# myfavouritekk/vdetlib

Measured on AMD Instinct MI355X. Metric: boxes/sec whole-node (NMS+temporal-conv+link), 300f×10k-box synth; mAP parity, higher is better.
Workload: dtype f32; 1 GPU; configs[1]+[2]: 1 video/GPU, 300 frames x 10000 boxes x 200 classes; per-(frame,class) NMS thresh 0.30 + temporal max-pool w=3 + 3-tap temporal convolution; greedy tubelets: 10 tracks/class (stop < 0.90), IoU-link >= 0.50, spatial max-pool IoU > 0.70 + completion + temporal max-pool; frames=300, boxes=10000, classes=200, scores=rand, parallelism=video-per-gpu x1, 4 distinct videos in flight per GPU

## Files before the change

vdetlib_amd/csrc/graphlists_kernels.hpp:

```cpp
#pragma once
#include <hip/hip_runtime.h>
#include <stdint.h>

#include "nms_kernels.hpp"

namespace vdet {

__device__ __forceinline__ int qreach_slot(const GroupDesc &gd, int g) { return ((gd.box_off >> 8) + g) * 4; }

__global__ __launch_bounds__(256) void row_classes_kernel(const float4 *__restrict__ xbox, const GroupDesc *__restrict__ groups,
                                                          const uint32_t *__restrict__ group_flags, float one_minus_t,
                                                          uint16_t *__restrict__ rowperm, float *__restrict__ qreach)
{
    __shared__ float sw[256];
    __shared__ float sreach[256];
    const int g = blockIdx.x, t = blockIdx.y, tid = threadIdx.x;
    if (!(group_flags[g] & kFlagRegular)) return;
    const GroupDesc gd = groups[g];
    if (t * 256 >= gd.nbox) return;
    const int s = t * 256 + tid;
    const bool valid = s < gd.nbox;
    float wd = 3.0e38f, reach = -3.0e38f;
    if (valid) { const float4 b = xbox[gd.box_off + s]; wd = b.z - b.x; reach = b.x + one_minus_t * ((b.z - b.x) + 1.0f) * 1.001f + 1.0f; }
    sw[tid] = wd;
    __syncthreads();
    int rank = 0;
    for (int j = 0; j < 256; ++j) { const float o = sw[j]; rank += (o < wd || (o == wd && j < tid)) ? 1 : 0; }
    if (valid) rowperm[gd.box_off + t * 256 + rank] = (uint16_t)s;
    sreach[rank] = reach;
    __syncthreads();
    float rc = sreach[tid];
#pragma unroll
    for (int d = 32; d > 0; d >>= 1) rc = fmaxf(rc, __shfl_xor(rc, d, 64));
    if ((tid & 63) == 0) qreach[qreach_slot(gd, g) + 4 * t + (tid >> 6)] = rc;
}

struct ListItem { int32_t group; int32_t tq; };

struct GraphListsParams {
    const float4 *xbox;
    const uint16_t *xord;
    const GroupDesc *groups;
    const uint32_t *group_flags;
    const ListItem *items;
    int nitems;
    float t32, one_minus_t;
    uint32_t *row_deg;
    const float2 *reach_table;
    const uint16_t *rowperm;
    const float *qreach;
    uint16_t *adj;
    uint32_t slot_cap;
    int *status;
    int over_bits;
    uint32_t trash_off;
};

__device__ __forceinline__ void emit_half(uint16_t *__restrict__ adj, uint32_t h, uint32_t boff, const uint16_t *ids, uint32_t *lpos,
                                          const uint16_t myid)
{
    constexpr int kSlots = 4;
// ... 187 lines not shown
```

vdetlib_amd/csrc/nms_kernels.hpp:

```cpp
#pragma once
#include <hip/hip_runtime.h>
#include <stdint.h>

namespace vdet {

struct GroupDesc {
    int32_t box_off;
    int32_t nbox;
    int64_t bits_off;
};

__device__ __host__ __forceinline__ int64_t bit_word(int nbox, int v, int c)
{
    const int W = (nbox + 63) >> 6;
    return ((int64_t)(v >> 6) * W + c) * 64 + (v & 63);
}
__host__ __device__ __forceinline__ int64_t bit_words_of_group(int nbox)
{
    const int64_t W = (nbox + 63) >> 6;
    return W * W * 64;
}

struct TileDesc {
    int32_t group;
// ... 760 lines not shown

struct ProblemRef { int g, N, rb; int64_t sbase, sstride, obase; };

__device__ __forceinline__ ProblemRef decode_problem(int mode, int p, int B, int C, const GroupDesc *groups)
{
    ProblemRef r;
    if (mode == 0) { r.g = p / C; const int c = p - r.g * C; r.sbase = (int64_t)r.g * B * C + c; r.sstride = C; r.obase = (int64_t)p * B; }
    else if (mode == 1 || mode == 3) { r.g = p / C; r.sbase = (int64_t)p * B; r.sstride = 1; r.obase = (int64_t)p * B; }
    else { r.g = p; r.sbase = groups[p].box_off; r.sstride = 1; r.obase = groups[p].box_off; }
    r.N = groups[r.g].nbox;
    r.rb = groups[r.g].box_off;
    return r;
}

__device__ __forceinline__ int xcd_problem(int bid, int nblocks)
{
    const int per = nblocks >> 3;
    return (bid & 7) * per + (bid >> 3);
}

__device__ __forceinline__ unsigned long long match8(uint32_t d, bool valid)
{
    unsigned long long peers = __ballot(valid);
#pragma unroll
    for (int b = 0; b < 8; ++b) {
        const bool bit = (d >> b) & 1u;
        const unsigned long long m = __ballot(valid && bit);
        peers &= bit ? m : ~m;
    }
    return peers;
}

template <int BLOCK, int CPW, bool ARANK>
__device__ __forceinline__ void lsd_sort_problem(const SortParams &prm, const int p, unsigned char *smem)
{
    constexpr int NW = BLOCK / 64;
    uint16_t *keys0 = reinterpret_cast<uint16_t *>(smem);
    uint16_t *src = reinterpret_cast<uint16_t *>(smem + prm.lds_idxa_off);
    uint16_t *dst = reinterpret_cast<uint16_t *>(smem + prm.lds_idxb_off);
    uint32_t *bases = reinterpret_cast<uint32_t *>(smem + prm.lds_base_off);
    uint32_t *tot = bases + NW * 256;
    __shared__ uint32_t swt[4];

    const int tid = threadIdx.x, lane = tid & 63, w = tid >> 6;
    const ProblemRef pr = decode_problem(prm.mode, p, prm.B, prm.C, prm.groups);
    const int N = pr.N;

    if (tid == 0) tot[256] = 0;
    __syncthreads();
    uint32_t nx = 0;
    uint32_t khi[(CPW + 1) / 2];
#pragma unroll
    for (int k = 0; k < (CPW + 1) / 2; ++k) khi[k] = 0xFFFFFFFFu;
    uint32_t raw[CPW];
    uint32_t exb[CPW];
    {
        const int lastv = max(N - 1, 0);
        if (prm.keys) {
#pragma unroll
            for (int k = 0; k < CPW; ++k) raw[k] = prm.keys[pr.sbase + min(tid + k * BLOCK, lastv)];
        } else {
#pragma unroll
            for (int k = 0; k < CPW; ++k) raw[k] = __float_as_uint(prm.scores[pr.sbase + (int64_t)min(tid + k * BLOCK, lastv) * pr.sstride]);
        }
#pragma unroll
        for (int k = 0; k < CPW; ++k) exb[k] = 0u;
        if (prm.excl) {
#pragma unroll
            for (int k = 0; k < CPW; ++k) exb[k] = prm.excl[pr.rb + min(tid + k * BLOCK, lastv)];
        }
    }
#pragma unroll
    for (int k = 0; k < CPW; ++k) {
        const int v = tid + k * BLOCK;
        if (v < N) {
            uint32_t ik;
            bool x = false;
            if (prm.keys) {
                const uint32_t kk = raw[k];
                ik = ~kk;
                x = (kk == 0u);
            } else {
                const float sc = __uint_as_float(raw[k]);
                ik = ~score_key(sc);
                if (prm.use_thr && !(sc > prm.thr)) x = true;
            }
            if (exb[k]) x = true;
            if (x) { ik = 0xFFFFFFFFu; ++nx; }
            keys0[v] = (uint16_t)(ik & 0xFFFFu);
            khi[k >> 1] = (k & 1) ? ((khi[k >> 1] & 0x0000FFFFu) | (ik & 0xFFFF0000u))
                                  : ((khi[k >> 1] & 0xFFFF0000u) | (ik >> 16));
            src[v] = (uint16_t)(N - 1 - v);
        }
    }
    if (nx) atomicAdd(&tot[256], nx);
    __syncthreads();
    const int ncand = N - (int)tot[256];

    const int nchunks = (N + 63) >> 6;
    const int c0 = w * CPW;

    for (int pass = 0; pass < 4; ++pass) {
        const int shift = (pass & 1) * 8;
        if (pass == 2) {
#pragma unroll
            for (int k = 0; k < CPW; ++k) {
                const int v = tid + k * BLOCK;
                if (v < N) keys0[v] = (uint16_t)((k & 1) ? (khi[k >> 1] >> 16) : (khi[k >> 1] & 0xFFFFu));
            }
        }
        for (int i = tid; i < NW * 256; i += BLOCK) bases[i] = 0;
        __syncthreads();
        uint32_t ra[CPW];
        uint32_t rl[CPW];
        bool peel_on = false;
#pragma unroll
        for (int ch = 0; ch < CPW; ++ch) {
            const int q = (c0 + ch) * 64 + lane;
            const bool valid = (c0 + ch) < nchunks && q < N;
            const uint32_t i = valid ? src[q] : 0u;
            const uint32_t d = valid ? (((uint32_t)keys0[i] >> shift) & 255u) : 0u;
            ra[ch] = i | (d << 16);
            if (ARANK) {
                uint32_t r = 0u;
                bool pending = valid;
#pragma unroll
                for (int peel = 0; peel < 2; ++peel) {
                    if (ch > 0 && !peel_on) break;
                    const unsigned long long rem = __ballot(pending);
                    if (rem) {
                        const int l0 = __ffsll((unsigned long long)rem) - 1;
// ... 30 lines not shown
#pragma unroll
            for (int ww = 0; ww < NW; ++ww) dsum += bases[ww * 256 + tid];
            dincl = dsum;
#define VDET_SCAN_STEP(CTRL, ROWMASK) dincl += (uint32_t)__builtin_amdgcn_update_dpp(0, (int)dincl, CTRL, ROWMASK, 0xf, false);
            VDET_SCAN_STEP(0x111, 0xf) VDET_SCAN_STEP(0x112, 0xf) VDET_SCAN_STEP(0x114, 0xf) VDET_SCAN_STEP(0x118, 0xf)
            VDET_SCAN_STEP(0x142, 0xa) VDET_SCAN_STEP(0x143, 0xc)
#undef VDET_SCAN_STEP
            if (lane == 63) swt[w] = dincl;
        }
        __syncthreads();
        if (tid < 256) {
            uint32_t run = dincl - dsum;
            for (int k = 0; k < w; ++k) run += swt[k];
#pragma unroll
            for (int ww = 0; ww < NW; ++ww) {
                const uint32_t c = bases[ww * 256 + tid];
                bases[ww * 256 + tid] = run;
                run += c;
            }
        }
        __syncthreads();
#pragma unroll
        for (int ch = 0; ch < CPW; ++ch) {
            const int q = (c0 + ch) * 64 + lane;
            const bool valid = (c0 + ch) < nchunks && q < N;
            if (valid) {
                const uint32_t d = ra[ch] >> 16;
                dst[bases[w * 256 + d] + rl[ch]] = (uint16_t)(ra[ch] & 0xFFFFu);
            }
        }
        __syncthreads();
        uint16_t *t = src; src = dst; dst = t;
    }
    int ncand_out = ncand;
    if (prm.topk > 0 && ncand > prm.topk) {
        const int k = prm.topk;
        if (w == 0) {
            auto key_at = [&](int q) -> uint32_t {
                const int i = src[q];
                if (prm.keys) return prm.keys[pr.sbase + i];
                return score_key(prm.scores[pr.sbase + (int64_t)i * pr.sstride]);
            };
            const uint32_t kk = key_at(k - 1);
            int a = k - 1, b = k;
            for (;;) {
                const int q = a - 1 - lane;
                const bool eq = q >= 0 && key_at(q) == kk;
                const unsigned long long m = __ballot(eq);
                const int n = m == ~0ull ? 64 : (__ffsll((unsigned long long)~m) - 1);
                a -= n;
                if (n < 64) break;
            }
            for (;;) {
                const int q = b + lane;
                const bool eq = q < ncand && key_at(q) == kk;
                const unsigned long long m = __ballot(eq);
                const int n = m == ~0ull ? 64 : (__ffsll((unsigned long long)~m) - 1);
                b += n;
                if (n < 64) break;
            }
            const int nsel = k - a, s0 = b - nsel;
            if (s0 > a)
                for (int t = 0; t < nsel; t += 64) {
                    const bool v = t + lane < nsel;
                    const uint16_t e = v ? src[s0 + t + lane] : (uint16_t)0;
                    __builtin_amdgcn_fence(__ATOMIC_ACQ_REL, "wavefront");
// ... 574 lines not shown
```

vdetlib_amd/csrc/vdet_capi.hip:

```cpp
#include <hip/hip_runtime.h>
#include <atomic>
#include <chrono>

#include <algorithm>
#include <cmath>
#include <cstdarg>
#include <cstdio>
#include <cstdlib>
#include <cstring>
#include <string>
#include <vector>

#include "../../include/vdet_hip.h"
#include "nms_kernels.hpp"
#include "binsort_kernels.hpp"
#include "small_kernels.hpp"
#include "detnms_kernels.hpp"
#include "fused_kernels.hpp"
#include "adjrows_kernels.hpp"
#include "graphlists_kernels.hpp"
#include "temporal_kernels.hpp"
#include "tubelet_kernels.hpp"
#include "track_kernels.hpp"
#include "batch_kernels.hpp"
#include "gemm_kernels.hpp"
#include "eval_kernels.hpp"
#include "tcn_kernels.hpp"
#include "interp_kernels.hpp"
#include "anchor_kernels.hpp"

using namespace vdet;

namespace {

struct DevBuf {
    void *p = nullptr;
    size_t cap = 0;
    hipError_t reserve(size_t bytes)
    {
        if (bytes <= cap) return hipSuccess;
        if (p) (void)hipFree(p);
        p = nullptr;
        cap = 0;
        size_t want = bytes + bytes / 4 + 256;
        hipError_t e = hipMalloc(&p, want);
        if (e != hipSuccess) {
            want = bytes;
            e = hipMalloc(&p, want);
// ... 70 lines not shown
    size_t bits_budget = (size_t)1 << 30;
    size_t max_lds = 160 * 1024;
    int n_cu = 256;
    DevBuf boxes, scores, keys, excl, frames, groups, tiles, bits, rowz, rowmeta, groupz, adj, comp, origidx,
        out64, trk_frames, trk_boxes, b1, b2, iou_out, order, ncand, keepidx, keepcnt, gflags, pairs, tkeys, tstate, visited, heads, xkeys, xord, wmeta, wmeta16, reachtab, rowperm, qreach, ditems, striptot, stripoff, xncand, xbox, xbox16, xord16, xcum, xinfo, tmp[8];
    bool timing = false;
    bool timing_accumulate = false;
    std::vector<std::pair<hipEvent_t, hipEvent_t>> ev_pool;
    std::vector<int> ev_stage;
    size_t ev_used = 0;
    float last_ms[ST_COUNT] = {0};
    int last_launches[ST_COUNT] = {0};
    bool sort_attr_set = false;
    bool cache_enabled = false;
    struct PrepKey { const void *boxes = nullptr; int64_t F = 0, B = 0; float t32 = 0; ListsKey lists; } prep;
    bool graph_valid = false, lists_valid = false;
    struct KeySrc { const void *scores = nullptr; int64_t F = 0, B = 0, C = 0; int use_thr = 0; float thr = 0; } keysrc;
    bool keys_valid = false;
    bool vpass_attr_set = false;
    bool index_valid = false; const void *index_boxes = nullptr; int64_t index_F = 0, index_B = 0;
    bool all_regular = false;
    bool wave_transpose = false;
    bool no_lazy = false;
    bool no_index = false;
    bool force_general = false;
    bool atomic_rank = false;
    bool small_lists = true;
    bool adj_rows = true;
    bool direct_lists = true;
    uint32_t direct_cap = 384;
    int64_t direct_ntot = 0;
    unsigned long long direct_fixed = 0;
    bool no_fused = false;
    bool binsort = true;
    const std::vector<GroupDesc> *host_groups = nullptr;
    bool sym_built = false;
    NmsPlan vplan;
    bool vplan_valid = false;
    int64_t vplan_F = 0, vplan_B = 0;
    size_t vplan_budget = 0;
    long long n_host_syncs = 0;
    bool async_enabled = false;
    unsigned long long pool_hint = 0;
    bool topk_attr_set = false;
    float gt32 = 0.f;
    bool wmeta16_built = false;
    bool wmeta_built = false;
    bool last_sort_binned = false;
    StagedTab vidtab, segtab;
    DevBuf sortctl;
    DevBuf nover;
    DevBuf ordncand;
    DevBuf linkmemo, linkstats, linkwarm, linkorder, linkchains, linknodes, tracknode, rtodo;
    struct NodeKey { const void *tracks = nullptr, *boxes = nullptr; int64_t F = 0, B = 0, C = 0; int T = 0; double nms_thres = 0; } nodekey;
    bool nodes_valid = false;
    void *fused_in = nullptr, *fused_out = nullptr;
    void *fused_in_dev = nullptr, *fused_out_dev = nullptr;
    void *fbatch_in = nullptr, *fbatch_out = nullptr, *fbatch_in_dev = nullptr, *fbatch_out_dev = nullptr;
    size_t fbatch_in_cap = 0, fbatch_out_cap = 0;
    bool fbatch_attr = false;
    size_t dyn_lds_max = 0;
    DevBuf ev_tab, ev_dtp, ev_dsc, ev_dslot, ev_bcnt, ev_boff, ev_key[2], ev_val[2], ev_hist;
    DevBuf tcn_x, tcn_frames, tcn_base, tcn_len, tcn_scratch;
    StagedTab tcn_params, tcn_foff, tcn_ovtab;
    bool tcn_tiled = false;
    bool tcn_global = false;
// ... 133 lines not shown
        if (gd.nbox < 2) { gd.bits_off = 0; continue; }
        const size_t words = (size_t)bit_words_of_group(gd.nbox);
        if (cur && cur + words > budget_words) {
            pl.batch_tiles.push_back({t0, (int)pl.tiles.size()});
            pl.batch_pairs.push_back({p0, (int)pl.pairs.size()});
            pl.batch_ditems.push_back({d0, (int)pl.ditems.size()});
            t0 = (int)pl.tiles.size();
            p0 = (int)pl.pairs.size();
            d0 = (int)pl.ditems.size();
            pl.bits_words_max = std::max(pl.bits_words_max, cur);
            cur = 0;
        }
        gd.bits_off = (int64_t)cur;
        cur += words;
        const int nrt = (gd.nbox + kRowsPerTile - 1) / kRowsPerTile;
        for (int rt = 0; rt < nrt; ++rt) pl.tiles.push_back({(int32_t)g, rt});
        for (int rt = 0; rt < nrt; ++rt)
            for (int ct = rt; ct < nrt; ++ct) pl.pairs.push_back({(int32_t)g, (int16_t)rt, (int16_t)ct});
        for (int q = 3; q >= 0; --q)
            for (int rt = 0; rt < nrt; ++rt) pl.ditems.push_back({(int32_t)g, (int32_t)(4 * rt + q)});
    }
    if ((int)pl.tiles.size() > t0) {
        pl.batch_tiles.push_back({t0, (int)pl.tiles.size()});
        pl.batch_pairs.push_back({p0, (int)pl.pairs.size()});
        pl.batch_ditems.push_back({d0, (int)pl.ditems.size()});
    }
    pl.bits_words_max = std::max(pl.bits_words_max, cur);
    (void)c;
    return VDET_OK;
}

int sort_groups_by_keys(vdet_ctx *c, int G, int nmax, int64_t ntot);

int build_frame_index(vdet_ctx *c, const float4 *d_boxes, int64_t ntot, int64_t G, int nmax)
{
    if (c->cache_enabled && c->index_valid && c->index_boxes == d_boxes && c->index_F == G && c->index_B == ntot) return VDET_OK;
    c->index_valid = false;
    HIPCHK(c, c->xkeys.reserve((size_t)ntot * 4));
    HIPCHK(c, c->xord.reserve((size_t)ntot * 2));
    HIPCHK(c, c->xncand.reserve((size_t)G * 4));
    HIPCHK(c, c->xbox.reserve((size_t)ntot * 16));
    HIPCHK(c, c->xbox16.reserve((size_t)(ntot + G + 4) * 8));
    HIPCHK(c, c->xord16.reserve((size_t)(ntot + G + 4) * 2));
    HIPCHK(c, c->xcum.reserve((size_t)G * 257 * 4));
    HIPCHK(c, c->xinfo.reserve((size_t)G * 16));
    StageTimer tm(c, ST_OTHER);
    hipLaunchKernelGGL(xkey_kernel, dim3((unsigned)((ntot + 255) / 256)), dim3(256), 0, c->stream, d_boxes,
                       c->xkeys.as<uint32_t>(), ntot);
    int rc = sort_groups_by_keys(c, (int)G, nmax, ntot);
    if (rc) return rc;
    hipLaunchKernelGGL(frame_index_kernel, dim3((unsigned)G), dim3(256), 0, c->stream, d_boxes, c->groups.as<GroupDesc>(),
                       c->xord.as<uint16_t>(), c->xbox.as<float4>(), c->xcum.as<uint32_t>(), c->xinfo.as<float>(),
                       c->gflags.as<uint32_t>(), c->xbox16.as<uint2>(), c->xord16.as<uint16_t>());
    HIPCHK(c, hipGetLastError());
    c->index_valid = true; c->index_boxes = d_boxes; c->index_F = G; c->index_B = ntot;
    return VDET_OK;
}

FrameIndex frame_index_of(vdet_ctx *c)
{
    return FrameIndex{c->xbox.as<float4>(), c->xord.as<uint16_t>(), c->xcum.as<uint32_t>(), c->xinfo.as<float>(),
                      c->xbox16.as<uint2>(), c->xord16.as<uint16_t>(), 0};
}

NmsPlan &volume_plan(vdet_ctx *c, int64_t F, int64_t B)
{
    if (c->vplan_F == F && c->vplan_B == B && c->vplan_budget == c->bits_budget && !c->vplan.groups.empty()) return c->vplan;
    (void)host_sync(c);
    c->graph_valid = c->lists_valid = c->index_valid = c->nodes_valid = false;
    c->vplan = NmsPlan();
    c->vplan.groups.resize((size_t)F);
    for (int64_t f = 0; f < F; ++f) c->vplan.groups[(size_t)f] = {(int32_t)(f * B), (int32_t)B, 0};
    make_plan(c, c->vplan);
    c->vplan_F = F; c->vplan_B = B; c->vplan_budget = c->bits_budget;
    c->vplan_valid = false;
    return c->vplan;
}

int volume_groups(vdet_ctx *c, int64_t F, int64_t B)
{
    NmsPlan &pl = volume_plan(c, F, B);
    c->host_groups = &pl.groups;
    HIPCHK(c, c->groups.reserve((size_t)F * sizeof(GroupDesc)));
    if (!c->vplan_valid)
        HIPCHK(c, hipMemcpyAsync(c->groups.p, pl.groups.data(), (size_t)F * sizeof(GroupDesc), hipMemcpyHostToDevice, c->stream));
    return VDET_OK;
}

// ... 111 lines not shown
        if (!pl.ditems.empty())
            HIPCHK(c, hipMemcpyAsync(c->ditems.p, pl.ditems.data(), pl.ditems.size() * sizeof(ListItem),
                                     hipMemcpyHostToDevice, c->stream));
        HIPCHK(c, hipMemcpyAsync(c->groups.p, pl.groups.data(), G * sizeof(GroupDesc), hipMemcpyHostToDevice, c->stream));
        if (!pl.tiles.empty())
            HIPCHK(c, hipMemcpyAsync(c->tiles.p, pl.tiles.data(), pl.tiles.size() * sizeof(TileDesc),
                                     hipMemcpyHostToDevice, c->stream));
        c->vplan_valid = volume;
    }
    auto direct_now = [&]() {
        return c->direct_lists && c->adj_rows && c->wave_transpose && pl.nmax > 384 && t32 > 1e-30f && t32 < INFINITY && !c->force_general &&
               (size_t)8 * pl.nmax + 24 * 1024 <= c->max_lds && ((unsigned long long)pl.ntot + 1ull) * c->direct_cap * 2ull + 512ull <= 0xFFFFFFFFull;
    };
    auto fixed_pool = [&]() { return direct_now() ? (unsigned long long)pl.ntot * c->direct_cap + std::max<unsigned long long>(c->direct_cap, 128) : 0ull; };
    unsigned long long min_pool = fixed_pool() + (unsigned long long)pl.ntot * (direct_now() ? 1 : 32);
    const bool async = volume && c->async_enabled && c->pool_hint > 0;
    if (async) {
        const unsigned long long dyn_hint = c->pool_hint > fixed_pool() ? c->pool_hint - fixed_pool() : 0ull;
        const unsigned long long want = std::max(min_pool, fixed_pool() + dyn_hint + dyn_hint / 2);
        if (c->adj.cap < want * 2) HIPCHK(c, c->adj.reserve((size_t)want * 2 + 4096));
    } else {
        Counters h0;
        HIPCHK(c, hipMemcpyAsync(&h0, c->d_cnt, sizeof h0, hipMemcpyDeviceToHost, c->stream));
        HIPCHK(c, host_sync(c));
        if (h0.status && !c->latched) c->latched = translate_status(c, h0.status);
        if (h0.eindex && !c->latched) c->latched = fail(c, VDET_EINDEX, "list index out of range");
        if (c->adj.cap < min_pool * 2) HIPCHK(c, c->adj.reserve((size_t)min_pool * 2 + 4096));
    }

    for (int attempt = 0; attempt < 3; ++attempt) {
        const bool direct = direct_now();
        min_pool = fixed_pool() + (unsigned long long)pl.ntot * (direct ? 1 : 32);
        if (!async && c->adj.cap < min_pool * 2) HIPCHK(c, c->adj.reserve((size_t)min_pool * 2 + 4096));
        HIPCHK(c, hipMemsetAsync(c->rowz.p, 0, (size_t)pl.ntot * 4, c->stream));
        HIPCHK(c, hipMemsetAsync(c->rowmeta.p, 0, (size_t)pl.ntot * 8, c->stream));
        HIPCHK(c, hipMemsetAsync(c->groupz.p, 0, G * 4, c->stream));
        if (async) {
            hipLaunchKernelGGL(fold_pool_kernel, dim3(1), dim3(1), 0, c->stream, c->d_cnt);
            HIPCHK(c, hipMemsetAsync((char *)c->d_cnt + kPerBuildOff, 0, sizeof(Counters) - kPerBuildOff, c->stream));
        }
        else HIPCHK(c, hipMemsetAsync(c->d_cnt, 0, sizeof(Counters), c->stream));
        c->direct_ntot = direct ? pl.ntot : 0;
        c->direct_fixed = fixed_pool();
        if (direct) hipLaunchKernelGGL(pool_start_kernel, dim3(1), dim3(1), 0, c->stream, &c->d_cnt->pool_used, fixed_pool());
        const int pool_bits = async ? (kStPool | kStPoolAsync) : kStPool;
        const unsigned long long pool_cap = (c->adj.cap - 2048) / 2;
        const bool use_sym = t32 > 1e-30f && t32 < INFINITY && !c->force_general &&
                             (size_t)8 * pl.nmax + 24 * 1024 <= c->max_lds;
        c->sym_built = use_sym;
        c->wmeta_built = use_sym;
        if (c->wmeta_built) HIPCHK(c, c->wmeta.reserve((size_t)pl.ntot * sizeof(WalkMeta)));
        if (c->wmeta_built && c->adj_rows && pl.nmax > 384) HIPCHK(c, c->wmeta16.reserve((size_t)pl.ntot * sizeof(uint4)));
        if (use_sym) {
            {
                StageTimer tm(c, ST_OTHER);
                hipLaunchKernelGGL(frame_flags_kernel, dim3((unsigned)G), dim3(256), 0, c->stream, d_boxes,
                                   c->groups.as<GroupDesc>(), c->gflags.as<uint32_t>(), &c->d_cnt->irregular);
            }
            if (!volume) c->index_valid = false;
            const int rci = build_frame_index(c, d_boxes, pl.ntot, (int64_t)G, pl.nmax);
            if (rci) return rci;
            HIPCHK(c, c->reachtab.reserve((size_t)(pl.ntot / 64 + (int64_t)G + 2) * sizeof(float2)));
            {
                StageTimer tm(c, ST_OTHER);
                hipLaunchKernelGGL(reach_table_kernel, dim3((unsigned)G), dim3(256), 0, c->stream, c->xbox.as<float4>(),
                                   c->groups.as<GroupDesc>(), c->gflags.as<uint32_t>(), one_minus_t, c->reachtab.as<float2>());
                if (direct) {
                    HIPCHK(c, c->rowperm.reserve((size_t)pl.ntot * 2 + 1024));
                    HIPCHK(c, c->qreach.reserve((size_t)(pl.ntot / 256 + (int64_t)G + 2) * 4 * sizeof(float)));
                    hipLaunchKernelGGL(row_classes_kernel, dim3((unsigned)G, (unsigned)((pl.nmax + 255) / 256)), dim3(256), 0, c->stream,
                                       c->xbox.as<float4>(), c->groups.as<GroupDesc>(), c->gflags.as<uint32_t>(), one_minus_t,
                                       c->rowperm.as<uint16_t>(), c->qreach.as<float>());
                }
            }
        } else {
            c->index_valid = false;
        }
        if (direct && !pl.ditems.empty()) {
            StageTimer tm(c, ST_IOU_BITS);
            GraphListsParams gp;
            gp.xbox = c->xbox.as<float4>(); gp.xord = c->xord.as<uint16_t>(); gp.groups = c->groups.as<GroupDesc>();
            gp.group_flags = c->gflags.as<uint32_t>(); gp.items = c->ditems.as<ListItem>(); gp.nitems = (int)pl.ditems.size();
            gp.t32 = t32; gp.one_minus_t = one_minus_t; gp.row_deg = c->rowz.as<uint32_t>(); gp.reach_table = c->reachtab.as<float2>();
            gp.rowperm = c->rowperm.as<uint16_t>(); gp.qreach = c->qreach.as<float>(); gp.adj = c->adj.as<uint16_t>();
            gp.slot_cap = c->direct_cap; gp.status = &c->d_cnt->status; gp.over_bits = pool_bits | kStDirect;
            gp.trash_off = (uint32_t)((unsigned long long)pl.ntot * c->direct_cap * 2ull);
// ... 608 lines not shown
    if (hipGetDeviceCount(&ndev) != hipSuccess || ndev <= 0) {
        delete c;
        return VDET_EHIP;
    }
    if (device < 0) {
        if (hipGetDevice(&device) != hipSuccess) { delete c; return VDET_EHIP; }
    }
    if (device >= ndev || hipSetDevice(device) != hipSuccess) { delete c; return VDET_EINVAL; }
    c->device = device;
    hipDeviceProp_t prop;
    if (hipGetDeviceProperties(&prop, device) == hipSuccess) {
        c->n_cu = prop.multiProcessorCount > 0 ? prop.multiProcessorCount : 256;
        if (strncmp(prop.gcnArchName, "gfx950", 6) != 0) c->max_lds = 64 * 1024;
    }
    if (const char *e = getenv("VDET_FORCE_GENERAL")) c->force_general = atoi(e) != 0;
    if (const char *e = getenv("VDET_BITS_BUDGET_MB")) {
        const long mb = atol(e);
        if (mb > 0) c->bits_budget = (size_t)mb << 20;
    }
    if (hipStreamCreateWithFlags(&c->own_stream, hipStreamNonBlocking) != hipSuccess ||
        hipMalloc((void **)&c->d_cnt, sizeof(Counters)) != hipSuccess) {
        delete c;
        return VDET_EHIP;
    }
    c->stream = c->own_stream;
    (void)hipMemsetAsync(c->d_cnt, 0, sizeof(Counters), c->stream);
    if (const char *e = getenv("VDET_NO_INDEX")) c->no_index = atoi(e) != 0;
    if (const char *e = getenv("VDET_NO_LAZY")) c->no_lazy = atoi(e) != 0;
    if (const char *e = getenv("VDET_NO_FUSED")) c->no_fused = atoi(e) != 0;
    if (const char *e = getenv("VDET_ADJ_ROWS")) c->adj_rows = atoi(e) != 0;
    if (const char *e = getenv("VDET_DIRECT_LISTS")) c->direct_lists = atoi(e) != 0;
    if (const char *e = getenv("VDET_DIRECT_CAP")) { const int v = atoi(e); if (v >= 8 && v <= 32760) c->direct_cap = (uint32_t)(v & ~7); }
    if (const char *e = getenv("VDET_BINSORT")) c->binsort = atoi(e) != 0;
    if (const char *e = getenv("VDET_SMALL_LISTS")) c->small_lists = atoi(e) != 0;
    if (const char *e = getenv("VDET_TCN_TILED")) c->tcn_tiled = atoi(e) != 0;
    if (const char *e = getenv("VDET_TCN_GLOBAL")) c->tcn_global = atoi(e) != 0;
    {
        const int npat = 4096;
        std::vector<uint8_t> pats((size_t)npat * 64);
        uint32_t rs = 12345u;
        auto rnd = [&]() { rs = rs * 1664525u + 1013904223u; return rs >> 8; };
        for (int t = 0; t < npat; ++t) {
            const int kind = t % 8;
            const int nd = kind == 0 ? 1 : kind == 1 ? 2 : kind == 2 ? 3 : kind == 3 ? 8 : kind == 4 ? 32 : kind == 5 ? 64 : kind == 6 ? 200 : 254;
            for (int l = 0; l < 64; ++l) {
                uint8_t d = (uint8_t)(rnd() % nd);
                if (kind == 7 && (rnd() & 3) == 0) d = 255;
                if (t % 16 == 9) d = (uint8_t)((l * (1 + t % 7)) % nd);
                pats[(size_t)t * 64 + l] = d;
            }
        }
        bool ok = false;
        DevBuf pb;
        if (pb.reserve(pats.size()) == hipSuccess &&
            hipMemcpyAsync(pb.p, pats.data(), pats.size(), hipMemcpyHostToDevice, c->stream) == hipSuccess) {
            hipLaunchKernelGGL(lds_atomic_order_probe, dim3(256), dim3(64), 0, c->stream, pb.as<uint8_t>(), npat,
                               &c->d_cnt->status);
            Counters h;
            if (hipMemcpyAsync(&h, c->d_cnt, sizeof h, hipMemcpyDeviceToHost, c->stream) == hipSuccess &&
                host_sync(c) == hipSuccess)
                ok = (h.status == 0);
        }
        pb.release();
        (void)hipMemsetAsync(c->d_cnt, 0, sizeof(Counters), c->stream);
        c->atomic_rank = ok;
        if (const char *e = getenv("VDET_ATOMIC_RANK")) c->atomic_rank = c->atomic_rank && atoi(e) != 0;
// ... 63 lines not shown
int vdet_reset_stream(vdet_ctx *c)
{
    if (!c) return VDET_EINVAL;
    c->stream = c->own_stream;
    return VDET_OK;
}

const char *vdet_last_error(vdet_ctx *c) { return c ? c->err.c_str() : "null context"; }

int vdet_set_cache(vdet_ctx *c, int enable)
{
    if (!c) return VDET_EINVAL;
    c->cache_enabled = enable != 0;
    c->graph_valid = c->lists_valid = c->index_valid = c->keys_valid = c->nodes_valid = false;
    return VDET_OK;
}

int vdet_invalidate(vdet_ctx *c)
{
    if (!c) return VDET_EINVAL;
    c->graph_valid = c->lists_valid = c->index_valid = c->keys_valid = c->nodes_valid = false;
    return VDET_OK;
}

int vdet_query(vdet_ctx *c, int what)
{
    if (!c) return VDET_EINVAL;
    if (what == 0) return c->atomic_rank ? 1 : 0;
    if (what == 1) return c->n_cu;
    if (what == 2) return c->all_regular ? 1 : 0;
    if (what == 3) return c->wave_transpose ? 1 : 0;
    if (what == 8) return (int)std::min<long long>(c->n_host_syncs, 0x7FFFFFFF);
    if (what == 10) return (int)std::min<long long>(c->tcn_params.uploads, 0x7FFFFFFF);
    if (what == 9) {
        if (!c->last_sort_binned || !c->sortctl.p) return -1;
        BinSortCtl h{};
        if (hipMemcpyAsync(&h, c->sortctl.p, sizeof h, hipMemcpyDeviceToHost, c->stream) != hipSuccess || host_sync(c) != hipSuccess) return VDET_EHIP;
        return h.nfail;
    }
    if (what >= 4 && what <= 7) {
        unsigned int h[4] = {0, 0, 0, 0};
        if (!c->linkstats.p) return 0;
        if (hipMemcpyAsync(h, c->linkstats.p, 16, hipMemcpyDeviceToHost, c->stream) != hipSuccess ||
            host_sync(c) != hipSuccess) return VDET_EHIP;
        return (int)std::min<unsigned int>(h[what - 4], 0x7FFFFFFFu);
    }
    return VDET_EINVAL;
}

int vdet_set_timing(vdet_ctx *c, int enable)
{
    if (!c) return VDET_EINVAL;
    c->timing = enable != 0;
    c->timing_accumulate = enable == 2;
    c->ev_used = 0;
    return VDET_OK;
}

int vdet_last_timing_ms(vdet_ctx *c, float *out16)
{
    float *out8 = out16;
    if (!c || !out8) return VDET_EINVAL;
    HIPCHK(c, host_sync(c));
    for (int i = 0; i < ST_COUNT; ++i) { c->last_ms[i] = 0; c->last_launches[i] = 0; }
    for (size_t i = 0; i < c->ev_used; ++i) {
        float ms = 0;
// ... 1739 lines not shown
```

Baseline: 332.5 million boxes/s.

## Fuse per-frame index build, flags, memsets and row ordering into one prep kernel

Adds a frame_prep_kernel with one 1024-thread block per frame. It computes validity and u16 flags, radix-sorts boxes by x in LDS, writes the sorted xbox/xord/xbox16, the bucket histogram prefix, the reach table, and the rowperm/qreach width ranks. The same kernel zeroes rowz, rowmeta and groupz and does the pool-start/fold bookkeeping, replacing several separate kernels and memsets. The goal is to cut launch count and the repeated global re-reads of boxes, at the cost of large LDS use per block and possibly lower occupancy. The row_classes_kernel rank loop now also runs only over valid entries.

```diff
diff --git a/vdetlib_amd/csrc/frameprep_kernels.hpp b/vdetlib_amd/csrc/frameprep_kernels.hpp
--- /dev/null
+++ b/vdetlib_amd/csrc/frameprep_kernels.hpp
@@ -0,0 +1,212 @@
+#pragma once
+#include <hip/hip_runtime.h>
+#include <stdint.h>
+
+#include "graphlists_kernels.hpp"
+#include "nms_kernels.hpp"
+
+namespace vdet {
+
+constexpr int kPrepBlock = 1024;
+constexpr int kPrepHistWords = 272;
+
+struct FramePrepParams {
+    const float4 *boxes;
+    const GroupDesc *groups;
+    uint32_t *group_flags;
+    int *n_irregular;
+    uint16_t *xord; float4 *xbox; uint32_t *xcum; float *xinfo; uint2 *xbox16; uint16_t *xord16;
+    float2 *reachtab;
+    uint16_t *rowperm; float *qreach;
+    uint32_t *rowz; uint2 *rowmeta; uint32_t *groupz;
+    unsigned long long *pool_used, *pool_max;
+    unsigned long long pool_start;
+    int fold;
+    float one_minus_t;
+    int lds_keys_off, lds_idxb_off, lds_base_off;
+};
+
+__host__ __device__ inline size_t frame_prep_lds(int nmax, int *keys_off, int *idxb_off, int *base_off)
+{
+    const size_t idx = (((size_t)2 * (size_t)(nmax > 1 ? nmax : 1)) + 15) & ~(size_t)15;
+    const size_t widths = (size_t)4 * (((size_t)nmax + 255) & ~(size_t)255);
+    const size_t base = idx + (2 * idx > widths ? 2 * idx : widths);
+    if (keys_off) *keys_off = (int)idx;
+    if (idxb_off) *idxb_off = (int)(2 * idx);
+    if (base_off) *base_off = (int)base;
+    return base + (size_t)4 * ((kPrepBlock / 64) * 256 + 256 + 4);
+}
+
+template <int CPW, bool ARANK>
+__global__ __launch_bounds__(kPrepBlock) void frame_prep_kernel(const FramePrepParams prm)
+{
+    extern __shared__ __attribute__((aligned(16))) unsigned char smem[];
+    constexpr int BLOCK = kPrepBlock;
+    __shared__ float smin[BLOCK / 64], smax[BLOCK / 64], swm[BLOCK / 64];
+    __shared__ uint32_t swsum[4];
+    const int g = blockIdx.x, tid = threadIdx.x, lane = tid & 63, w = tid >> 6;
+    if (g == 0 && tid == 0) {
+        if (prm.fold && *prm.pool_used > *prm.pool_max) *prm.pool_max = *prm.pool_used;
+        *prm.pool_used = prm.pool_start;
+    }
+    const GroupDesc gd = prm.groups[g];
+    const int N = gd.nbox;
+    const int64_t fo = gd.box_off;
+    if (tid == 0) prm.groupz[g] = 0u;
+    if (N <= 0) {
+        if (tid == 0) prm.group_flags[g] = kFlagRegular | kFlagU16;
+        return;
+    }
+    const float4 *fb = prm.boxes + fo;
+    uint16_t *src = reinterpret_cast<uint16_t *>(smem);
+    uint16_t *keys0 = reinterpret_cast<uint16_t *>(smem + prm.lds_keys_off);
+    uint16_t *dst = reinterpret_cast<uint16_t *>(smem + prm.lds_idxb_off);
+    uint32_t *bases = reinterpret_cast<uint32_t *>(smem + prm.lds_base_off);
+
+    constexpr int LD = CPW < 6 ? CPW : 6;
+    uint32_t khi[(CPW + 1) / 2];
+#pragma unroll
+    for (int k = 0; k < (CPW + 1) / 2; ++k) khi[k] = 0xFFFFFFFFu;
+    int bad = 0, wide = 0;
+    float mn = 3.0e38f, mx = -3.0e38f, wm = 0.0f;
+    const float inf = __uint_as_float(0x7F800000u);
+#pragma unroll
+    for (int k0 = 0; k0 < CPW; k0 += LD) {
+        float4 bx[LD];
+#pragma unroll
+        for (int j = 0; j < LD; ++j)
+            if (k0 + j < CPW) bx[j] = fb[min(tid + (k0 + j) * BLOCK, N - 1)];
+#pragma unroll
+        for (int j = 0; j < LD; ++j) {
+            const int k = k0 + j < CPW ? k0 + j : CPW - 1;
+            const int v = tid + k * BLOCK;
+            if (k0 + j < CPW && v < N) {
+                const float4 b = bx[j];
+                const float bw = (b.z - b.x) + 1.0f, bh = (b.w - b.y) + 1.0f;
+                const float a = bw * bh;
+                const bool ok = fabsf(b.x) < inf && fabsf(b.y) < inf && fabsf(b.z) < inf && fabsf(b.w) < inf && bw > 0.0f && bh > 0.0f && a < inf;
+                bad |= ok ? 0 : 1;
+                const bool small = b.x == truncf(b.x) && b.y == truncf(b.y) && b.z == truncf(b.z) && b.w == truncf(b.w) &&
+                                   fmaxf(fmaxf(b.x, b.y), fmaxf(b.z, b.w)) <= 65535.0f &&
+                                   ((__float_as_uint(b.x) | __float_as_uint(b.y) | __float_as_uint(b.z) | __float_as_uint(b.w)) >> 31) == 0u;
+                wide |= small ? 0 : 1;
+                mn = fminf(mn, b.x); mx = fmaxf(mx, b.x); wm = fmaxf(wm, bw);
+                const uint32_t ik = score_key(b.x);
+                keys0[v] = (uint16_t)(ik & 0xFFFFu);
+                khi[k >> 1] = (k & 1) ? ((khi[k >> 1] & 0x0000FFFFu) | (ik & 0xFFFF0000u)) : ((khi[k >> 1] & 0xFFFF0000u) | (ik >> 16));
+                src[v] = (uint16_t)(N - 1 - v);
+                prm.rowz[fo + v] = 0u;
+                prm.rowmeta[fo + v] = make_uint2(0u, 0u);
+            }
+        }
+    }
+#pragma unroll
+    for (int d = 32; d > 0; d >>= 1) {
+        mn = fminf(mn, __shfl_xor(mn, d, 64)); mx = fmaxf(mx, __shfl_xor(mx, d, 64)); wm = fmaxf(wm, __shfl_xor(wm, d, 64));
+    }
+    if (lane == 0) { smin[w] = mn; smax[w] = mx; swm[w] = wm; }
+    const int any_bad = __syncthreads_or(bad);
+    const int any_wide = __syncthreads_or(wide);
+    const uint32_t fl = (any_bad ? 0u : kFlagRegular) | (any_wide ? 0u : kFlagU16);
+    if (tid == 0) {
+        prm.group_flags[g] = fl;
+        if (any_bad) atomicAdd(prm.n_irregular, 1);
+    }
+#pragma unroll
+    for (int i = 0; i < BLOCK / 64; ++i) { mn = fminf(mn, smin[i]); mx = fmaxf(mx, smax[i]); wm = fmaxf(wm, swm[i]); }
+    const float xmin = mn, xmax = mx;
+    const float scale = xmax > xmin ? 256.0f / (xmax - xmin) : 0.0f;
+
+    lsd_sort_passes<BLOCK, CPW, ARANK>(keys0, src, dst, bases, khi, N);
+
+    float *swd = reinterpret_cast<float *>(smem + prm.lds_keys_off);
+    uint32_t *hist = bases;
+    float *sreach = reinterpret_cast<float *>(bases + kPrepHistWords);
+    for (int i = tid; i < 257; i += BLOCK) hist[i] = 0u;
+    __syncthreads();
+    const bool regular = (fl & kFlagRegular) != 0u;
+    const bool u16 = prm.xbox16 && (fl & kFlagU16);
+    const int64_t p16 = pair_pos(fo + g);
+#pragma unroll
+    for (int k = 0; k < CPW; ++k) {
+        const int r = tid + k * BLOCK;
+        float4 b = make_float4(0.f, 0.f, 0.f, 0.f);
+        float reach = -3.0e38f;
+        if (r < N) {
+            const uint16_t o = src[r];
+            b = fb[o];
+            prm.xbox[fo + r] = b;
+            prm.xord[fo + r] = o;
+            if (u16) {
+                prm.xbox16[p16 + r] = make_uint2((uint32_t)b.x | ((uint32_t)b.y << 16), (uint32_t)b.z | ((uint32_t)b.w << 16));
+                prm.xord16[p16 + r] = o;
+            }
+            atomicAdd(&hist[xbucket(b.x, xmin, scale) + 1], 1u);
+            swd[r] = b.z - b.x;
+            reach = b.x + prm.one_minus_t * ((b.z - b.x) + 1.0f) * 1.001f + 1.0f;
+        }
+        const int cb = k * (BLOCK / 64) + w;
+        if (regular && cb * 64 < N) {
+#pragma unroll
+            for (int d = 32; d > 0; d >>= 1) reach = fmaxf(reach, __shfl_xor(reach, d, 64));
+            const float first = __shfl(b.x, 0, 64);
+            if (lane == 0) prm.reachtab[reach_slot(gd, g) + cb] = make_float2(reach, first);
+        }
+    }
+    __syncthreads();
+    {
+        uint32_t incl = 0u;
+        if (tid < 256) {
+            incl = hist[tid + 1];
+#pragma unroll
+            for (int d = 1; d < 64; d <<= 1) { const uint32_t o = __shfl_up(incl, d, 64); if (lane >= d) incl += o; }
+            if (lane == 63) swsum[w] = incl;
+        }
+        __syncthreads();
+        if (tid < 256) {
+            for (int i = 0; i < w; ++i) incl += swsum[i];
+            prm.xcum[(int64_t)g * 257 + tid + 1] = incl;
+        }
+        if (tid == 0) {
+            prm.xcum[(int64_t)g * 257] = 0u;
+            prm.xinfo[g * 4 + 0] = xmin; prm.xinfo[g * 4 + 1] = scale; prm.xinfo[g * 4 + 2] = wm; prm.xinfo[g * 4 + 3] = 0.0f;
+        }
+    }
+
+    if (!prm.rowperm || !regular) return;
+    const int grp = tid >> 8, pos = tid & 255;
+#pragma unroll
+    for (int k = 0; k < CPW; ++k) {
+        if (k * BLOCK < N) {
+            const int tile = grp + 4 * k, tb = tile * 256;
+            const int nv = min(256, N - tb);
+            int rank = pos;
+            float reach = -3.0e38f;
+            if (pos < nv) {
+                const float4 b = prm.xbox[fo + tb + pos];
+                reach = b.x + prm.one_minus_t * ((b.z - b.x) + 1.0f) * 1.001f + 1.0f;
+                const float wd = swd[tb + pos];
+                rank = 0;
+                for (int j = 0; j < nv; j += 4) {
+                    const float4 o = *reinterpret_cast<const float4 *>(swd + tb + j);
+                    rank += (o.x < wd || (o.x == wd && j < pos)) ? 1 : 0;
+                    rank += (j + 1 < nv && (o.y < wd || (o.y == wd && j + 1 < pos))) ? 1 : 0;
+                    rank += (j + 2 < nv && (o.z < wd || (o.z == wd && j + 2 < pos))) ? 1 : 0;
+                    rank += (j + 3 < nv && (o.w < wd || (o.w == wd && j + 3 < pos))) ? 1 : 0;
+                }
+                prm.rowperm[fo + tb + rank] = (uint16_t)(tb + pos);
+            }
+            if (nv > 0) sreach[grp * 256 + rank] = reach;
+            __syncthreads();
+            if (nv > 0) {
+                float rc = sreach[tid];
+#pragma unroll
+                for (int d = 32; d > 0; d >>= 1) rc = fmaxf(rc, __shfl_xor(rc, d, 64));
+                if (lane == 0) prm.qreach[qreach_slot(gd, g) + 4 * tile + (w & 3)] = rc;
+            }
+            __syncthreads();
+        }
+    }
+}
+
+}
diff --git a/vdetlib_amd/csrc/graphlists_kernels.hpp b/vdetlib_amd/csrc/graphlists_kernels.hpp
--- a/vdetlib_amd/csrc/graphlists_kernels.hpp
+++ b/vdetlib_amd/csrc/graphlists_kernels.hpp
@@ -20,13 +20,17 @@
     if (t * 256 >= gd.nbox) return;
     const int s = t * 256 + tid;
     const bool valid = s < gd.nbox;
-    float wd = 3.0e38f, reach = -3.0e38f;
+    float wd = 0.0f, reach = -3.0e38f;
     if (valid) { const float4 b = xbox[gd.box_off + s]; wd = b.z - b.x; reach = b.x + one_minus_t * ((b.z - b.x) + 1.0f) * 1.001f + 1.0f; }
     sw[tid] = wd;
     __syncthreads();
-    int rank = 0;
-    for (int j = 0; j < 256; ++j) { const float o = sw[j]; rank += (o < wd || (o == wd && j < tid)) ? 1 : 0; }
-    if (valid) rowperm[gd.box_off + t * 256 + rank] = (uint16_t)s;
+    const int nv = min(256, gd.nbox - t * 256);
+    int rank = tid;
+    if (valid) {
+        rank = 0;
+        for (int j = 0; j < nv; ++j) { const float o = sw[j]; rank += (o < wd || (o == wd && j < tid)) ? 1 : 0; }
+        rowperm[gd.box_off + t * 256 + rank] = (uint16_t)s;
+    }
     sreach[rank] = reach;
     __syncthreads();
     float rc = sreach[tid];
diff --git a/vdetlib_amd/csrc/nms_kernels.hpp b/vdetlib_amd/csrc/nms_kernels.hpp
--- a/vdetlib_amd/csrc/nms_kernels.hpp
+++ b/vdetlib_amd/csrc/nms_kernels.hpp
@@ -816,71 +816,12 @@
 }
 
 template <int BLOCK, int CPW, bool ARANK>
-__device__ __forceinline__ void lsd_sort_problem(const SortParams &prm, const int p, unsigned char *smem)
+__device__ __forceinline__ void lsd_sort_passes(uint16_t *keys0, uint16_t *&src, uint16_t *&dst, uint32_t *bases, const uint32_t (&khi)[(CPW + 1) / 2],
+                                                const int N)
 {
     constexpr int NW = BLOCK / 64;
-    uint16_t *keys0 = reinterpret_cast<uint16_t *>(smem);
-    uint16_t *src = reinterpret_cast<uint16_t *>(smem + prm.lds_idxa_off);
-    uint16_t *dst = reinterpret_cast<uint16_t *>(smem + prm.lds_idxb_off);
-    uint32_t *bases = reinterpret_cast<uint32_t *>(smem + prm.lds_base_off);
-    uint32_t *tot = bases + NW * 256;
     __shared__ uint32_t swt[4];
-
     const int tid = threadIdx.x, lane = tid & 63, w = tid >> 6;
-    const ProblemRef pr = decode_problem(prm.mode, p, prm.B, prm.C, prm.groups);
-    const int N = pr.N;
-
-    if (tid == 0) tot[256] = 0;
-    __syncthreads();
-    uint32_t nx = 0;
-    uint32_t khi[(CPW + 1) / 2];
-#pragma unroll
-    for (int k = 0; k < (CPW + 1) / 2; ++k) khi[k] = 0xFFFFFFFFu;
-    uint32_t raw[CPW];
-    uint32_t exb[CPW];
-    {
-        const int lastv = max(N - 1, 0);
-        if (prm.keys) {
-#pragma unroll
-            for (int k = 0; k < CPW; ++k) raw[k] = prm.keys[pr.sbase + min(tid + k * BLOCK, lastv)];
-        } else {
-#pragma unroll
-            for (int k = 0; k < CPW; ++k) raw[k] = __float_as_uint(prm.scores[pr.sbase + (int64_t)min(tid + k * BLOCK, lastv) * pr.sstride]);
-        }
-#pragma unroll
-        for (int k = 0; k < CPW; ++k) exb[k] = 0u;
-        if (prm.excl) {
-#pragma unroll
-            for (int k = 0; k < CPW; ++k) exb[k] = prm.excl[pr.rb + min(tid + k * BLOCK, lastv)];
-        }
-    }
-#pragma unroll
-    for (int k = 0; k < CPW; ++k) {
-        const int v = tid + k * BLOCK;
-        if (v < N) {
-            uint32_t ik;
-            bool x = false;
-            if (prm.keys) {
-                const uint32_t kk = raw[k];
-                ik = ~kk;
-                x = (kk == 0u);
-            } else {
-                const float sc = __uint_as_float(raw[k]);
-                ik = ~score_key(sc);
-                if (prm.use_thr && !(sc > prm.thr)) x = true;
-            }
-            if (exb[k]) x = true;
-            if (x) { ik = 0xFFFFFFFFu; ++nx; }
-            keys0[v] = (uint16_t)(ik & 0xFFFFu);
-            khi[k >> 1] = (k & 1) ? ((khi[k >> 1] & 0x0000FFFFu) | (ik & 0xFFFF0000u))
-                                  : ((khi[k >> 1] & 0xFFFF0000u) | (ik >> 16));
-            src[v] = (uint16_t)(N - 1 - v);
-        }
-    }
-    if (nx) atomicAdd(&tot[256], nx);
-    __syncthreads();
-    const int ncand = N - (int)tot[256];
-
     const int nchunks = (N + 63) >> 6;
     const int c0 = w * CPW;
 
@@ -977,6 +918,74 @@
         __syncthreads();
         uint16_t *t = src; src = dst; dst = t;
     }
+}
+
+template <int BLOCK, int CPW, bool ARANK>
+__device__ __forceinline__ void lsd_sort_problem(const SortParams &prm, const int p, unsigned char *smem)
+{
+    constexpr int NW = BLOCK / 64;
+    uint16_t *keys0 = reinterpret_cast<uint16_t *>(smem);
+    uint16_t *src = reinterpret_cast<uint16_t *>(smem + prm.lds_idxa_off);
+    uint16_t *dst = reinterpret_cast<uint16_t *>(smem + prm.lds_idxb_off);
+    uint32_t *bases = reinterpret_cast<uint32_t *>(smem + prm.lds_base_off);
+    uint32_t *tot = bases + NW * 256;
+    const int tid = threadIdx.x, lane = tid & 63, w = tid >> 6;
+    const ProblemRef pr = decode_problem(prm.mode, p, prm.B, prm.C, prm.groups);
+    const int N = pr.N;
+
+    if (tid == 0) tot[256] = 0;
+    __syncthreads();
+    uint32_t nx = 0;
+    uint32_t khi[(CPW + 1) / 2];
+#pragma unroll
+    for (int k = 0; k < (CPW + 1) / 2; ++k) khi[k] = 0xFFFFFFFFu;
+    uint32_t raw[CPW];
+    uint32_t exb[CPW];
+    {
+        const int lastv = max(N - 1, 0);
+        if (prm.keys) {
+#pragma unroll
+            for (int k = 0; k < CPW; ++k) raw[k] = prm.keys[pr.sbase + min(tid + k * BLOCK, lastv)];
+        } else {
+#pragma unroll
+            for (int k = 0; k < CPW; ++k) raw[k] = __float_as_uint(prm.scores[pr.sbase + (int64_t)min(tid + k * BLOCK, lastv) * pr.sstride]);
+        }
+#pragma unroll
+        for (int k = 0; k < CPW; ++k) exb[k] = 0u;
+        if (prm.excl) {
+#pragma unroll
+            for (int k = 0; k < CPW; ++k) exb[k] = prm.excl[pr.rb + min(tid + k * BLOCK, lastv)];
+        }
+    }
+#pragma unroll
+    for (int k = 0; k < CPW; ++k) {
+        const int v = tid + k * BLOCK;
+        if (v < N) {
+            uint32_t ik;
+            bool x = false;
+            if (prm.keys) {
+                const uint32_t kk = raw[k];
+                ik = ~kk;
+                x = (kk == 0u);
+            } else {
+                const float sc = __uint_as_float(raw[k]);
+                ik = ~score_key(sc);
+                if (prm.use_thr && !(sc > prm.thr)) x = true;
+            }
+            if (exb[k]) x = true;
+            if (x) { ik = 0xFFFFFFFFu; ++nx; }
+            keys0[v] = (uint16_t)(ik & 0xFFFFu);
+            khi[k >> 1] = (k & 1) ? ((khi[k >> 1] & 0x0000FFFFu) | (ik & 0xFFFF0000u))
+                                  : ((khi[k >> 1] & 0xFFFF0000u) | (ik >> 16));
+            src[v] = (uint16_t)(N - 1 - v);
+        }
+    }
+    if (nx) atomicAdd(&tot[256], nx);
+    __syncthreads();
+    const int ncand = N - (int)tot[256];
+
+    lsd_sort_passes<BLOCK, CPW, ARANK>(keys0, src, dst, bases, khi, N);
+
     int ncand_out = ncand;
     if (prm.topk > 0 && ncand > prm.topk) {
         const int k = prm.topk;
diff --git a/vdetlib_amd/csrc/vdet_capi.hip b/vdetlib_amd/csrc/vdet_capi.hip
--- a/vdetlib_amd/csrc/vdet_capi.hip
+++ b/vdetlib_amd/csrc/vdet_capi.hip
@@ -5,6 +5,7 @@
 #include <algorithm>
 #include <cmath>
 #include <cstdarg>
+#include <cstddef>
 #include <cstdio>
 #include <cstdlib>
 #include <cstring>
@@ -14,6 +15,7 @@
 #include "../../include/vdet_hip.h"
 #include "nms_kernels.hpp"
 #include "binsort_kernels.hpp"
+#include "frameprep_kernels.hpp"
 #include "small_kernels.hpp"
 #include "detnms_kernels.hpp"
 #include "fused_kernels.hpp"
@@ -150,6 +152,10 @@
     int64_t direct_ntot = 0;
     unsigned long long direct_fixed = 0;
     bool no_fused = false;
+    bool frame_prep = true;
+    bool prep_attr_set = false;
+    bool prep_fused = false;
+    size_t prep_static_lds = 0;
     bool binsort = true;
     const std::vector<GroupDesc> *host_groups = nullptr;
     bool sym_built = false;
@@ -349,18 +355,24 @@
 
 int sort_groups_by_keys(vdet_ctx *c, int G, int nmax, int64_t ntot);
 
-int build_frame_index(vdet_ctx *c, const float4 *d_boxes, int64_t ntot, int64_t G, int nmax)
-{
-    if (c->cache_enabled && c->index_valid && c->index_boxes == d_boxes && c->index_F == G && c->index_B == ntot) return VDET_OK;
-    c->index_valid = false;
-    HIPCHK(c, c->xkeys.reserve((size_t)ntot * 4));
+int reserve_frame_index(vdet_ctx *c, int64_t ntot, int64_t G)
+{
     HIPCHK(c, c->xord.reserve((size_t)ntot * 2));
-    HIPCHK(c, c->xncand.reserve((size_t)G * 4));
     HIPCHK(c, c->xbox.reserve((size_t)ntot * 16));
     HIPCHK(c, c->xbox16.reserve((size_t)(ntot + G + 4) * 8));
     HIPCHK(c, c->xord16.reserve((size_t)(ntot + G + 4) * 2));
     HIPCHK(c, c->xcum.reserve((size_t)G * 257 * 4));
     HIPCHK(c, c->xinfo.reserve((size_t)G * 16));
+    return VDET_OK;
+}
+
+int build_frame_index(vdet_ctx *c, const float4 *d_boxes, int64_t ntot, int64_t G, int nmax)
+{
+    if (c->cache_enabled && c->index_valid && c->index_boxes == d_boxes && c->index_F == G && c->index_B == ntot) return VDET_OK;
+    c->index_valid = false;
+    HIPCHK(c, c->xkeys.reserve((size_t)ntot * 4));
+    HIPCHK(c, c->xncand.reserve((size_t)G * 4));
+    if (const int rc = reserve_frame_index(c, ntot, G)) return rc;
     StageTimer tm(c, ST_OTHER);
     hipLaunchKernelGGL(xkey_kernel, dim3((unsigned)((ntot + 255) / 256)), dim3(256), 0, c->stream, d_boxes,
                        c->xkeys.as<uint32_t>(), ntot);
@@ -371,6 +383,36 @@
                        c->gflags.as<uint32_t>(), c->xbox16.as<uint2>(), c->xord16.as<uint16_t>());
     HIPCHK(c, hipGetLastError());
     c->index_valid = true; c->index_boxes = d_boxes; c->index_F = G; c->index_B = ntot;
+    return VDET_OK;
+}
+
+int frame_prep_variant(vdet_ctx *c, int nmax, const void **fn, size_t *lds)
+{
+    struct Variant { int cpw; const void *fn[2]; };
+#define VDET_FP(CP) {CP, {reinterpret_cast<const void *>(frame_prep_kernel<CP, false>), reinterpret_cast<const void *>(frame_prep_kernel<CP, true>)}}
+    static const Variant variants[] = {VDET_FP(2), VDET_FP(4), VDET_FP(10)};
+#undef VDET_FP
+    *fn = nullptr;
+    if (!c->frame_prep || nmax <= 384) return VDET_OK;
+    if (!c->prep_attr_set) {
+        size_t stat = 0;
+        for (const Variant &v : variants)
+            for (const void *f : v.fn) {
+                hipFuncAttributes fa;
+                HIPCHK(c, hipFuncGetAttributes(&fa, f));
+                stat = std::max(stat, (size_t)fa.sharedSizeBytes);
+            }
+        c->prep_static_lds = (stat + 15) & ~(size_t)15;
+        for (const Variant &v : variants)
+            for (const void *f : v.fn)
+                HIPCHK(c, hipFuncSetAttribute(f, hipFuncAttributeMaxDynamicSharedMemorySize, (int)(c->max_lds - c->prep_static_lds)));
+        c->prep_attr_set = true;
+    }
+    *lds = frame_prep_lds(nmax, nullptr, nullptr, nullptr);
+    if (*lds + c->prep_static_lds > c->max_lds) return VDET_OK;
+    const int need_cpw = ((nmax + 63) / 64 + kPrepBlock / 64 - 1) / (kPrepBlock / 64);
+    for (const Variant &v : variants)
+        if (v.cpw >= need_cpw) { *fn = v.fn[c->atomic_rank ? 1 : 0]; break; }
     return VDET_OK;
 }
 
@@ -548,26 +590,58 @@
         const bool direct = direct_now();
         min_pool = fixed_pool() + (unsigned long long)pl.ntot * (direct ? 1 : 32);
         if (!async && c->adj.cap < min_pool * 2) HIPCHK(c, c->adj.reserve((size_t)min_pool * 2 + 4096));
-        HIPCHK(c, hipMemsetAsync(c->rowz.p, 0, (size_t)pl.ntot * 4, c->stream));
-        HIPCHK(c, hipMemsetAsync(c->rowmeta.p, 0, (size_t)pl.ntot * 8, c->stream));
-        HIPCHK(c, hipMemsetAsync(c->groupz.p, 0, G * 4, c->stream));
-        if (async) {
+        const bool use_sym = t32 > 1e-30f && t32 < INFINITY && !c->force_general &&
+                             (size_t)8 * pl.nmax + 24 * 1024 <= c->max_lds;
+        const void *prep_fn = nullptr;
+        size_t prep_lds = 0;
+        if (use_sym && volume)
+            if (const int rcp = frame_prep_variant(c, pl.nmax, &prep_fn, &prep_lds)) return rcp;
+        c->prep_fused = prep_fn != nullptr;
+        if (!prep_fn) {
+            HIPCHK(c, hipMemsetAsync(c->rowz.p, 0, (size_t)pl.ntot * 4, c->stream));
+            HIPCHK(c, hipMemsetAsync(c->rowmeta.p, 0, (size_t)pl.ntot * 8, c->stream));
+            HIPCHK(c, hipMemsetAsync(c->groupz.p, 0, G * 4, c->stream));
+        }
+        if (async && prep_fn)
+            HIPCHK(c, hipMemsetAsync((char *)c->d_cnt + kPerBuildOff, 0, offsetof(Counters, pool_used) - kPerBuildOff, c->stream));
+        else if (async) {
             hipLaunchKernelGGL(fold_pool_kernel, dim3(1), dim3(1), 0, c->stream, c->d_cnt);
             HIPCHK(c, hipMemsetAsync((char *)c->d_cnt + kPerBuildOff, 0, sizeof(Counters) - kPerBuildOff, c->stream));
         }
         else HIPCHK(c, hipMemsetAsync(c->d_cnt, 0, sizeof(Counters), c->stream));
         c->direct_ntot = direct ? pl.ntot : 0;
         c->direct_fixed = fixed_pool();
-        if (direct) hipLaunchKernelGGL(pool_start_kernel, dim3(1), dim3(1), 0, c->stream, &c->d_cnt->pool_used, fixed_pool());
+        if (direct && !prep_fn) hipLaunchKernelGGL(pool_start_kernel, dim3(1), dim3(1), 0, c->stream, &c->d_cnt->pool_used, fixed_pool());
         const int pool_bits = async ? (kStPool | kStPoolAsync) : kStPool;
         const unsigned long long pool_cap = (c->adj.cap - 2048) / 2;
-        const bool use_sym = t32 > 1e-30f && t32 < INFINITY && !c->force_general &&
-                             (size_t)8 * pl.nmax + 24 * 1024 <= c->max_lds;
         c->sym_built = use_sym;
         c->wmeta_built = use_sym;
         if (c->wmeta_built) HIPCHK(c, c->wmeta.reserve((size_t)pl.ntot * sizeof(WalkMeta)));
         if (c->wmeta_built && c->adj_rows && pl.nmax > 384) HIPCHK(c, c->wmeta16.reserve((size_t)pl.ntot * sizeof(uint4)));
-        if (use_sym) {
+        if (prep_fn) {
+            c->index_valid = false;
+            if (const int rci = reserve_frame_index(c, pl.ntot, (int64_t)G)) return rci;
+            HIPCHK(c, c->reachtab.reserve((size_t)(pl.ntot / 64 + (int64_t)G + 2) * sizeof(float2)));
+            if (direct) {
+                HIPCHK(c, c->rowperm.reserve((size_t)pl.ntot * 2 + 1024));
+                HIPCHK(c, c->qreach.reserve((size_t)(pl.ntot / 256 + (int64_t)G + 2) * 4 * sizeof(float)));
+            }
+            FramePrepParams fp;
+            fp.boxes = d_boxes; fp.groups = c->groups.as<GroupDesc>(); fp.group_flags = c->gflags.as<uint32_t>();
+            fp.n_irregular = &c->d_cnt->irregular;
+            fp.xord = c->xord.as<uint16_t>(); fp.xbox = c->xbox.as<float4>(); fp.xcum = c->xcum.as<uint32_t>(); fp.xinfo = c->xinfo.as<float>();
+            fp.xbox16 = c->xbox16.as<uint2>(); fp.xord16 = c->xord16.as<uint16_t>();
+            fp.reachtab = c->reachtab.as<float2>();
+            fp.rowperm = direct ? c->rowperm.as<uint16_t>() : nullptr; fp.qreach = direct ? c->qreach.as<float>() : nullptr;
+            fp.rowz = c->rowz.as<uint32_t>(); fp.rowmeta = c->rowmeta.as<uint2>(); fp.groupz = c->groupz.as<uint32_t>();
+            fp.pool_used = &c->d_cnt->pool_used; fp.pool_max = &c->d_cnt->pool_max;
+            fp.pool_start = fixed_pool(); fp.fold = async ? 1 : 0; fp.one_minus_t = one_minus_t;
+            (void)frame_prep_lds(pl.nmax, &fp.lds_keys_off, &fp.lds_idxb_off, &fp.lds_base_off);
+            void *pargs[] = {&fp};
+            StageTimer tm(c, ST_OTHER);
+            HIPCHK(c, hipLaunchKernel(prep_fn, dim3((unsigned)G), dim3(kPrepBlock), pargs, prep_lds, c->stream));
+            c->index_valid = true; c->index_boxes = d_boxes; c->index_F = (int64_t)G; c->index_B = pl.ntot;
+        } else if (use_sym) {
             {
                 StageTimer tm(c, ST_OTHER);
                 hipLaunchKernelGGL(frame_flags_kernel, dim3((unsigned)G), dim3(256), 0, c->stream, d_boxes,
@@ -1242,6 +1316,7 @@
     if (const char *e = getenv("VDET_DIRECT_LISTS")) c->direct_lists = atoi(e) != 0;
     if (const char *e = getenv("VDET_DIRECT_CAP")) { const int v = atoi(e); if (v >= 8 && v <= 32760) c->direct_cap = (uint32_t)(v & ~7); }
     if (const char *e = getenv("VDET_BINSORT")) c->binsort = atoi(e) != 0;
+    if (const char *e = getenv("VDET_FRAME_PREP")) c->frame_prep = atoi(e) != 0;
     if (const char *e = getenv("VDET_SMALL_LISTS")) c->small_lists = atoi(e) != 0;
     if (const char *e = getenv("VDET_TCN_TILED")) c->tcn_tiled = atoi(e) != 0;
     if (const char *e = getenv("VDET_TCN_GLOBAL")) c->tcn_global = atoi(e) != 0;
@@ -1371,6 +1446,7 @@
     if (what == 3) return c->wave_transpose ? 1 : 0;
     if (what == 8) return (int)std::min<long long>(c->n_host_syncs, 0x7FFFFFFF);
     if (what == 10) return (int)std::min<long long>(c->tcn_params.uploads, 0x7FFFFFFF);
+    if (what == 11) return c->prep_fused ? 1 : 0;
     if (what == 9) {
         if (!c->last_sort_binned || !c->sortctl.p) return -1;
         BinSortCtl h{};
```

After: 325.5 million boxes/s. -2.1%, worse.
